# matter-labs/era-zkevm_test_harness

Measured on AMD Instinct MI355X. Metric: base-layer circuits/sec (2^20 rows); full-block synth wall-time 1/8 GPU, higher is better.
Workload: dtype u64 (Goldilocks, p = 2^64 - 2^32 + 1)

## Files before the change

### era_zkevm_test_harness_amd/csrc/ram_circuit_kernels.cuh

```cuda
#pragma once
#include "../../include/zkw_ram_circuit_spec.h"
#include "../../include/zkw_decommit_sorter_circuit_spec.h"
#include "../../include/zkw_events_sorter_circuit_spec.h"
#include "ram_kernels.cuh"
#include "public_input_kernels.cuh"
#include "closed_form_kernels.cuh"

namespace zkw {

struct SynthJob {
    const zkw_ram_instance* inst;
    const zkw_mem_query* sorted_q;
    const zkw_mem_query* unsorted_q;
    const u64* unsorted_caps;
    const u64* sorted_caps;
    const u64* u_mark;
    const u64* s_mark;
    const u64* challenges;
    const u64* lhs_z;
    const u64* rhs_z;
    u64 n_block;
    u64* trace;
    u32* hist;
    u32* nd_tiles;
    const u64* public_input;
    const zkw_ram_instance* first_inst;
    u32 tail_clean;
};

constexpr int ROW_SLOTS[RC_NUM_ROW_TYPES] = RC_ROW_NUM_SLOTS_INIT;
constexpr int ROW_LOOKUPS[RC_NUM_ROW_TYPES] = RC_ROW_NUM_LOOKUPS_INIT;
static_assert(ROW_SLOTS[RC_ROW_PU] == 133 && ROW_SLOTS[RC_ROW_PS] == 130, "Poseidon2 rows: 130 gate variables (+3 spare in PU)");
static_assert(ROW_LOOKUPS[RC_ROW_PU] == 12 && ROW_LOOKUPS[RC_ROW_PS] == 12 && ROW_LOOKUPS[RC_ROW_A] == 12 &&
              ROW_LOOKUPS[RC_ROW_B] == 12 && ROW_LOOKUPS[RC_ROW_C] == 8 && ROW_LOOKUPS[RC_ROW_D] == 0,
              "lookup cells per cycle (56) are hard-wired in the fill kernels");
constexpr int LOOKUPS_PER_CYCLE = 56;

__device__ __forceinline__ u64 inv_or_zero(u64 x) { return gl::canon(x) ? gl::inv(x) : 0; }

struct RegsIn {
    const u64* uh;
    const u64* sh;
    u32 len;
};
__device__ __forceinline__ RegsIn regs_in(const zkw_ram_instance* in) {
    RegsIn r;
    const bool start = in->start_flag != 0;
    r.uh = start ? in->unsorted_queue_initial_state.head : in->hidden_fsm_input.current_unsorted_queue_state.head;
    r.sh = start ? in->sorted_queue_initial_state.head : in->hidden_fsm_input.current_sorted_queue_state.head;
    r.len = start ? in->unsorted_queue_initial_state.length : in->hidden_fsm_input.current_unsorted_queue_state.length;
    return r;
}

#define TR(col, row) trace[(size_t)(col) * n_rows + (row)]

__device__ __forceinline__ void zero_gap_row(u64* trace, size_t n_rows, size_t row) {
    for (int col = 0; col < RC_G + RC_L; col++) TR(col, row) = 0;
}
__device__ __forceinline__ void zero_gap_row_n(u64* trace, size_t n_rows, size_t row, int n_cols) {
    for (int col = 0; col < n_cols; col++) TR(col, row) = 0;
}

__device__ __forceinline__ void hist_bytes(u32* sh_hist, u32 x) {
    atomicAdd(&sh_hist[x & 0xFF], 1u);
    atomicAdd(&sh_hist[(x >> 8) & 0xFF], 1u);
    atomicAdd(&sh_hist[(x >> 16) & 0xFF], 1u);
    atomicAdd(&sh_hist[x >> 24], 1u);
}
__device__ __forceinline__ void put_bytes(u64* trace, size_t n_rows, size_t row, int col0, u32 x) {
    TR(col0, row) = x & 0xFF;
    TR(col0 + 1, row) = (x >> 8) & 0xFF;
    TR(col0 + 2, row) = (x >> 16) & 0xFF;
    TR(col0 + 3, row) = x >> 24;
}
__device__ __forceinline__ void hist_flush(u32* sh_hist, u32* g_hist) {
    __syncthreads();
    for (int t = threadIdx.x; t < 256; t += blockDim.x)
        if (sh_hist[t]) atomicAdd(&g_hist[t], sh_hist[t]);
}

__device__ __forceinline__ void fill_flattened_poseidon(u64* trace, size_t n_rows, size_t row, u64 s[12]) {
    int pos = 0;
#pragma unroll
    for (int k = 0; k < 12; k++) TR(pos++, row) = gl::canon(s[k]);
    p2::external(s);
    int r = 0;
    for (int k = 0; k < P2_HALF_FULL_ROUNDS; k++, r++) {
        p2::full_round(s, r);
#pragma unroll
        for (int j = 0; j < 12; j++) TR(pos + j, row) = gl::canon(s[j]);
        pos += 12;
    }
    for (int k = 0; k < P2_PARTIAL_ROUNDS; k++, r++) {
        s[0] = gl::pow7(gl::add_canon(s[0], p2::rc_at(12 * r)));
        TR(pos++, row) = gl::canon(s[0]);
        p2::internal(s);
    }
    for (int k = 0; k < P2_HALF_FULL_ROUNDS; k++, r++) {
        p2::full_round(s, r);
#pragma unroll
        for (int j = 0; j < 12; j++) TR(pos + j, row) = gl::canon(s[j]);
        pos += 12;
    }
}

template <int SIDE>
static __device__ __forceinline__ void k_ram_fill_poseidon(const VB& vb, const SynthJob* __restrict__ jobs, u32 capacity,
                                                          size_t n_rows) {
    __shared__ u32 sh_hist[256];
    for (int t = threadIdx.x; t < 256; t += blockDim.x) sh_hist[t] = 0;
    __syncthreads();
    const SynthJob job = jobs[vb.y];
    const u32 i = vb.x * blockDim.x + threadIdx.x;
    if (i < capacity) {
        u64* trace = job.trace;
        const zkw_ram_instance* in = job.inst;
        const size_t first = in->first_item, m = in->num_items;
        const bool can_pop = i < m;
        const size_t row = (size_t)(SIDE == 0 ? RC_ROW_PU : RC_ROW_PS) * RC_REGION_STRIDE(capacity) + i;
        const zkw_mem_query* qs = SIDE == 0 ? job.unsorted_q : job.sorted_q;
        const u64* caps = SIDE == 0 ? job.unsorted_caps : job.sorted_caps;
        u64 s[12];
        if (can_pop) {
            encode_raw_query(load_raw_query(qs + first + i), s);
        } else {
#pragma unroll
            for (int k = 0; k < 8; k++) s[k] = 0;
        }
        const RegsIn ri = regs_in(in);
        const u64* prev_cap = i == 0 ? (SIDE == 0 ? ri.uh : ri.sh) + 8 : caps + 4 * (first + (i - 1 < m ? i - 1 : m - 1));
#pragma unroll
        for (int k = 0; k < 4; k++) s[8 + k] = prev_cap[k];
        fill_flattened_poseidon(trace, n_rows, row, s);
        zkw_mem_query q;
        memset(&q, 0, sizeof q);
        if (can_pop) q = job.sorted_q[first + i];
        if (SIDE == 0) {
            TR(RC_PU_idx, row) = q.index; TR(RC_PU_v0, row) = q.value[0]; TR(RC_PU_v1, row) = q.value[1];
            put_bytes(trace, n_rows, row, RC_PU_idx_b0, q.index);
            put_bytes(trace, n_rows, row, RC_PU_v0_b0, q.value[0]);
            put_bytes(trace, n_rows, row, RC_PU_v1_b0, q.value[1]);
            hist_bytes(sh_hist, q.index); hist_bytes(sh_hist, q.value[0]); hist_bytes(sh_hist, q.value[1]);
        } else {
            if (!job.tail_clean) for (int c = 130; c < RC_G; c++) TR(c, row) = 0;
            put_bytes(trace, n_rows, row, RC_PS_ts_b0, q.timestamp);
            put_bytes(trace, n_rows, row, RC_PS_page_b0, q.page);
            put_bytes(trace, n_rows, row, RC_PS_v4_b0, q.value[4]);
            hist_bytes(sh_hist, q.timestamp); hist_bytes(sh_hist, q.page); hist_bytes(sh_hist, q.value[4]);
        }
        if (!job.tail_clean) for (int c = RC_G + 12; c < RC_G + RC_L; c++) TR(c, row) = 0;
    } else if (i < RC_REGION_STRIDE(capacity)) {
        if (!job.tail_clean) zero_gap_row(job.trace, n_rows, (size_t)(SIDE == 0 ? RC_ROW_PU : RC_ROW_PS) * RC_REGION_STRIDE(capacity) + i);
    }
    hist_flush(sh_hist, job.hist);
}

struct CycleCtx {
    bool can_pop;
    zkw_mem_query q, pq;
    u64 eu[8], es[8];
    u64 p_val[5];
    u32 p_ptr;
};

__device__ __forceinline__ void load_query(const zkw_mem_query* src, zkw_mem_query& dst) {
    const uint4* s = reinterpret_cast<const uint4*>(src);
    uint4* d = reinterpret_cast<uint4*>(&dst);
    d[0] = s[0]; d[1] = s[1]; d[2] = s[2];
}

__device__ __forceinline__ void cycle_ctx(const SynthJob& job, u32 i, CycleCtx& c, bool want_eu) {
    const zkw_ram_instance* in = job.inst;
    const size_t first = in->first_item, m = in->num_items;
    c.can_pop = i < m;
    memset(&c.q, 0, sizeof c.q);
    memset(&c.pq, 0, sizeof c.pq);
#pragma unroll
    for (int k = 0; k < 8; k++) { c.eu[k] = 0; c.es[k] = 0; }
    if (c.can_pop) {
        load_query(job.sorted_q + first + i, c.q);
        encode_mem_query(c.q, c.es);
        if (want_eu) encode_raw_query(load_raw_query(job.unsorted_q + first + i), c.eu);
    }
    if (i == 0) {
        const zkw_ram_fsm& f = in->hidden_fsm_input;
        c.pq.timestamp = f.previous_sorting_key[0]; c.pq.index = f.previous_sorting_key[1]; c.pq.page = f.previous_sorting_key[2];
        for (int k = 0; k < 8; k++) c.pq.value[k] = f.previous_value[k];
        c.pq.value_is_pointer = f.previous_is_ptr ? 1 : 0;
    } else if (i - 1 < m) {
        load_query(job.sorted_q + first + i - 1, c.pq);
    }
    u64 pe[8];
    encode_mem_query(c.pq, pe);
#pragma unroll
    for (int k = 0; k < 5; k++) c.p_val[k] = pe[3 + k];
    c.p_ptr = c.pq.value_is_pointer ? 1 : 0;
}

__device__ __forceinline__ u64 acc_before(const u64* z, size_t first, size_t m, u32 i, u64 fsm_in) {
    return i == 0 ? fsm_in : z[first + (i - 1 < m ? i - 1 : m - 1)];
}

static __device__ __forceinline__ void k_ram_fill_A(const VB& vb, const SynthJob* __restrict__ jobs, u32 capacity, size_t n_rows) {
    __shared__ u32 sh_hist[256];
    sh_hist[threadIdx.x] = 0;
    __syncthreads();
    const SynthJob job = jobs[vb.y];
    const u32 i = vb.x * blockDim.x + threadIdx.x;
    const u64* lhs_z_all = job.lhs_z;
    const u64* rhs_z_all = job.rhs_z;
    const size_t n_total = job.n_block;
    if (i < capacity) {
        u64* trace = job.trace;
        const zkw_ram_instance* in = job.inst;
        const size_t first = in->first_item, m = in->num_items, row = (size_t)RC_ROW_A * RC_REGION_STRIDE(capacity) + i;
        CycleCtx c;
        cycle_ctx(job, i, c, true);
        const u64 rw = c.q.rw_flag ? 1 : 0, ptr = c.q.value_is_pointer ? 1 : 0;
#pragma unroll
        for (int k = 0; k < 8; k++) { TR(RC_A_eu0 + k, row) = c.eu[k]; TR(RC_A_ts + k, row) = c.es[k]; }
        for (int r = 0; r < 2; r++) {
            const u64* ch = job.challenges + 9 * r;
            u64 lc = ch[8], rc = ch[8];
#pragma unroll
            for (int k = 0; k < 8; k++) {
                lc = gl::add(lc, gl::mul(c.eu[k], ch[k]));
                rc = gl::add(rc, gl::mul(c.es[k], ch[k]));
            }
            const u64 pl = acc_before(lhs_z_all + (size_t)r * n_total, first, m, i, in->hidden_fsm_input.lhs_accumulator[r]);
            const u64 pr = acc_before(rhs_z_all + (size_t)r * n_total, first, m, i, in->hidden_fsm_input.rhs_accumulator[r]);
            const u64 nl = gl::canon(gl::mul(pl, lc)), nr = gl::canon(gl::mul(pr, rc));
            const int o = r * (RC_A_lc1 - RC_A_lc0);
#pragma unroll
            for (int k = 1; k < 9; k++) TR(RC_A_G_c0_1 + (k - 1) + r * (RC_A_G_c1_1 - RC_A_G_c0_1), row) = ch[k];
            TR(RC_A_lc0 + o, row) = gl::canon(lc); TR(RC_A_P_lhs0 + o, row) = pl; TR(RC_A_nl0 + o, row) = nl;
            TR(RC_A_lhs0 + o, row) = c.can_pop ? nl : pl;
            TR(RC_A_rc0 + o, row) = gl::canon(rc); TR(RC_A_P_rhs0 + o, row) = pr; TR(RC_A_nr0 + o, row) = nr;
            TR(RC_A_rhs0 + o, row) = c.can_pop ? nr : pr;
        }
        TR(RC_A_rw, row) = rw; TR(RC_A_ptr, row) = ptr; TR(RC_A_idx, row) = c.q.index;
        TR(RC_A_v2, row) = c.q.value[2]; TR(RC_A_v3, row) = c.q.value[3]; TR(RC_A_v0, row) = c.q.value[0];
        TR(RC_A_v5_b3c, row) = c.q.value[5] >> 24; TR(RC_A_can_pop, row) = c.can_pop ? 1 : 0;
        put_bytes(trace, n_rows, row, RC_A_v2_b0, c.q.value[2]);
        put_bytes(trace, n_rows, row, RC_A_v3_b0, c.q.value[3]);
        put_bytes(trace, n_rows, row, RC_A_v5_b0, c.q.value[5]);
        hist_bytes(sh_hist, c.q.value[2]); hist_bytes(sh_hist, c.q.value[3]); hist_bytes(sh_hist, c.q.value[5]);
        constexpr int NA = ROW_SLOTS[RC_ROW_A];
        if (!job.tail_clean) {
            for (int col = NA; col < RC_G; col++) TR(col, row) = 0;
            for (int col = RC_G + 12; col < RC_G + RC_L; col++) TR(col, row) = 0;
        }
    } else if (i < RC_REGION_STRIDE(capacity)) {
        if (!job.tail_clean) zero_gap_row(job.trace, n_rows, (size_t)RC_ROW_A * RC_REGION_STRIDE(capacity) + i);
    }
    hist_flush(sh_hist, job.hist);
}

static __device__ __forceinline__ void k_ram_fill_B(const VB& vb, const SynthJob* __restrict__ jobs, u32 capacity, size_t n_rows) {
    __shared__ u32 sh_hist[256];
    sh_hist[threadIdx.x] = 0;
    __syncthreads();
    const SynthJob job = jobs[vb.y];
    const u32 i = vb.x * blockDim.x + threadIdx.x;
    if (i < capacity) {
        u64* trace = job.trace;
        const size_t row = (size_t)RC_ROW_B * RC_REGION_STRIDE(capacity) + i;
        CycleCtx c;
        cycle_ctx(job, i, c, false);
        put_bytes(trace, n_rows, row, RC_B_v6_b0, c.q.value[6]);
        put_bytes(trace, n_rows, row, RC_B_v7_b0, c.q.value[7]);
        TR(RC_B_es4, row) = c.es[4]; TR(RC_B_v1, row) = c.q.value[1]; TR(RC_B_v5_b3c, row) = c.q.value[5] >> 24;
        TR(RC_B_es5, row) = c.es[5]; TR(RC_B_v2, row) = c.q.value[2];
        TR(RC_B_es6, row) = c.es[6]; TR(RC_B_v3, row) = c.q.value[3];
        const u32 d0 = c.q.timestamp - c.pq.timestamp;
        TR(RC_B_d0, row) = d0; put_bytes(trace, n_rows, row, RC_B_d0_b0, d0);
        TR(RC_B_bw0, row) = c.q.timestamp < c.pq.timestamp ? 1 : 0;
        TR(RC_B_ts, row) = c.q.timestamp; TR(RC_B_P_ts, row) = c.pq.timestamp;
        hist_bytes(sh_hist, c.q.value[6]); hist_bytes(sh_hist, c.q.value[7]); hist_bytes(sh_hist, d0);
        constexpr int NB = ROW_SLOTS[RC_ROW_B];
        if (!job.tail_clean) {
            for (int col = NB; col < RC_G; col++) TR(col, row) = 0;
            for (int col = RC_G + 12; col < RC_G + RC_L; col++) TR(col, row) = 0;
        }
    } else if (i < RC_REGION_STRIDE(capacity)) {
        if (!job.tail_clean) zero_gap_row(job.trace, n_rows, (size_t)RC_ROW_B * RC_REGION_STRIDE(capacity) + i);
    }
    hist_flush(sh_hist, job.hist);
}

__device__ __forceinline__ bool nd_flag(bool can_pop, const zkw_mem_query& q) {
    return can_pop && q.timestamp == 0 && q.page == RC_HEAP_PAGE && q.rw_flag && !q.value_is_pointer;
}

static __device__ __forceinline__ void k_ram_nd_tiles(const VB& vb, const SynthJob* __restrict__ jobs, u32 capacity) {
    __shared__ u32 sh[4];
    const SynthJob job = jobs[vb.y];
    const u32 i = vb.x * blockDim.x + threadIdx.x;
    const zkw_ram_instance* in = job.inst;
    bool f = false;
    if (i < capacity && i < in->num_items) {
        zkw_mem_query q;
        load_query(job.sorted_q + in->first_item + i, q);
        f = nd_flag(true, q);
    }
    u32 cnt = __popcll(__ballot(f));
    if ((threadIdx.x & 63) == 0) sh[threadIdx.x >> 6] = cnt;
    __syncthreads();
    if (threadIdx.x == 0) job.nd_tiles[vb.x] = sh[0] + sh[1] + sh[2] + sh[3];
}
static __device__ __forceinline__ void k_ram_nd_scan(const VB& vb, const SynthJob* __restrict__ jobs, int n_jobs, u32 n_tiles) {
    u32* t = jobs[vb.x].nd_tiles;
    const int lane = threadIdx.x;
    u32 acc = 0;
    for (u32 base = 0; base < n_tiles; base += 64) {
        const u32 k = base + lane;
        const u32 v = k < n_tiles ? t[k] : 0;
        u32 incl = v;
        for (int off = 1; off < 64; off <<= 1) {
            const u32 up = __shfl_up(incl, off);
            if (lane >= off) incl += up;
        }
        if (k < n_tiles) t[k] = acc + incl - v;
        acc += __shfl(incl, 63);
    }
}

static __device__ __forceinline__ void k_ram_fill_C(const VB& vb, const SynthJob* __restrict__ jobs, u32 capacity, size_t n_rows) {
    __shared__ u32 sh_hist[256];
    __shared__ u32 sh_wave[4];
    sh_hist[threadIdx.x] = 0;
    __syncthreads();
    const SynthJob job = jobs[vb.y];
    const u32 i = vb.x * blockDim.x + threadIdx.x;
    const bool live = i < capacity;
    CycleCtx c;
    c.can_pop = false;
    bool nd = false;
    if (live) {
        cycle_ctx(job, i, c, false);
        nd = nd_flag(c.can_pop, c.q);
    }
    const unsigned long long bal = __ballot(nd);
    const int lane = threadIdx.x & 63, wave = threadIdx.x >> 6;
    if (lane == 0) sh_wave[wave] = __popcll(bal);
    __syncthreads();
    u32 before = __popcll(bal & ((1ull << lane) - 1));
    for (int w = 0; w < wave; w++) before += sh_wave[w];
    if (live) {
        u64* trace = job.trace;
        const zkw_ram_instance* in = job.inst;
        const size_t row = (size_t)RC_ROW_C * RC_REGION_STRIDE(capacity) + i;
        const u64 rw = c.q.rw_flag ? 1 : 0, ptr = c.q.value_is_pointer ? 1 : 0;
        const u64 bw0 = c.q.timestamp < c.pq.timestamp ? 1 : 0;
        const u64 t1 = (u64)c.pq.index + bw0, bw1 = (u64)c.q.index < t1 ? 1 : 0;
        const u32 d1 = (u32)((u64)c.q.index - t1);
        const u64 t2 = (u64)c.pq.page + bw1, bw2 = (u64)c.q.page < t2 ? 1 : 0;
        const u32 d2 = (u32)((u64)c.q.page - t2);
        TR(RC_C_d1, row) = d1; put_bytes(trace, n_rows, row, RC_C_d1_b0, d1);
        TR(RC_C_d2, row) = d2; put_bytes(trace, n_rows, row, RC_C_d2_b0, d2);
        hist_bytes(sh_hist, d1); hist_bytes(sh_hist, d2);
        TR(RC_C_bw1, row) = bw1; TR(RC_C_bw2, row) = bw2; TR(RC_C_bw0, row) = bw0;
        TR(RC_C_idx, row) = c.q.index; TR(RC_C_P_idx, row) = c.pq.index;
        TR(RC_C_page, row) = c.q.page; TR(RC_C_P_page, row) = c.pq.page;
        TR(RC_C_can_pop, row) = c.can_pop ? 1 : 0;
        u64 x[14];
        x[0] = gl::canon(gl::sub(c.q.index, c.pq.index));
        x[1] = gl::canon(gl::sub(c.q.page, c.pq.page));
        const u64 val[5] = {c.es[3], c.es[4], c.es[5], c.es[6], c.es[7]};
#pragma unroll
        for (int k = 0; k < 5; k++) { x[2 + k] = gl::canon(gl::sub(val[k], c.p_val[k])); x[7 + k] = val[k]; }
        x[12] = c.q.timestamp;
        x[13] = gl::canon(gl::sub(c.q.page, RC_HEAP_PAGE));
        u64 pre[14], acc = 1;
#pragma unroll
        for (int k = 0; k < 14; k++) { pre[k] = acc; acc = gl::mul(acc, x[k] ? x[k] : 1); }
        u64 inv = gl::inv(acc), w[14];
#pragma unroll
        for (int k = 13; k >= 0; k--) {
            w[k] = x[k] ? gl::canon(gl::mul(inv, pre[k])) : 0;
            inv = gl::mul(inv, x[k] ? x[k] : 1);
        }
        const u64 z_idx = x[0] == 0, z_page = x[1] == 0, same = z_idx & z_page;
        TR(RC_C_w_idx, row) = w[0]; TR(RC_C_z_idx, row) = z_idx;
        TR(RC_C_w_page, row) = w[1]; TR(RC_C_z_page, row) = z_page; TR(RC_C_same, row) = same;
        const int C_VAL[5] = {RC_C_es3, RC_C_es4, RC_C_es5, RC_C_es6, RC_C_v4};
        const int C_PVAL[5] = {RC_C_P_es3, RC_C_P_es4, RC_C_P_es5, RC_C_P_es6, RC_C_P_v4};
        const int C_WEQ[5] = {RC_C_w_eq0, RC_C_w_eq1, RC_C_w_eq2, RC_C_w_eq3, RC_C_w_eq4};
        const int C_ZEQ[5] = {RC_C_z_eq0, RC_C_z_eq1, RC_C_z_eq2, RC_C_z_eq3, RC_C_z_eq4};
        const int C_WZ[5] = {RC_C_w_z0, RC_C_w_z1, RC_C_w_z2, RC_C_w_z3, RC_C_w_z4};
        const int C_ZZ[5] = {RC_C_z_z0, RC_C_z_z1, RC_C_z_z2, RC_C_z_z3, RC_C_z_z4};
        u64 zeq[5], zz[5];
#pragma unroll
        for (int k = 0; k < 5; k++) {
            zeq[k] = x[2 + k] == 0; zz[k] = x[7 + k] == 0;
            TR(C_VAL[k], row) = val[k]; TR(C_PVAL[k], row) = c.p_val[k];
            TR(C_WEQ[k], row) = w[2 + k]; TR(C_ZEQ[k], row) = zeq[k];
            TR(C_WZ[k], row) = w[7 + k]; TR(C_ZZ[k], row) = zz[k];
        }
        const u64 peq = ptr == c.p_ptr, eq_a = zeq[0] & zeq[1] & zeq[2], value_equal = eq_a & zeq[3] & zeq[4] & peq;
        const u64 zz_a = zz[0] & zz[1] & zz[2], all_zero = zz_a & zz[3] & zz[4] & (1 - ptr);
        TR(RC_C_ptr, row) = ptr; TR(RC_C_P_ptr, row) = c.p_ptr; TR(RC_C_peq, row) = peq;
        TR(RC_C_eq_a, row) = eq_a; TR(RC_C_value_equal, row) = value_equal;
        TR(RC_C_zz_a, row) = zz_a; TR(RC_C_all_zero, row) = all_zero; TR(RC_C_rw, row) = rw;
        TR(RC_C_ts, row) = c.q.timestamp; TR(RC_C_w_ts, row) = w[12]; TR(RC_C_z_ts, row) = x[12] == 0;
        TR(RC_C_w_heap, row) = w[13]; TR(RC_C_z_heap, row) = x[13] == 0; TR(RC_C_nd, row) = nd ? 1 : 0;
        const u64 p_cnt = (u64)in->hidden_fsm_input.num_nondeterministic_writes + job.nd_tiles[vb.x] + before;
        TR(RC_C_P_cnt, row) = p_cnt; TR(RC_C_cnt, row) = p_cnt + (nd ? 1 : 0);
        constexpr int NC = ROW_SLOTS[RC_ROW_C];
        if (!job.tail_clean) {
            for (int col = NC; col < RC_G; col++) TR(col, row) = 0;
            for (int col = RC_G + 8; col < RC_G + RC_L; col++) TR(col, row) = 0;
        }
    } else if (i < RC_REGION_STRIDE(capacity)) {
        if (!job.tail_clean) zero_gap_row(job.trace, n_rows, (size_t)RC_ROW_C * RC_REGION_STRIDE(capacity) + i);
    }
    if (vb.x == 0 && threadIdx.x == 0)
        for (int l = 5; l < 8; l++) { hist_bytes(sh_hist, job.inst->hidden_fsm_input.previous_value[l]); hist_bytes(sh_hist, job.inst->hidden_fsm_output.previous_value[l]); }
    hist_flush(sh_hist, job.hist);
}

__device__ __forceinline__ void ram_boundary_block(const SynthJob& job, u32 capacity, size_t n_rows);
constexpr int RC_D_TILES = 4;
// ... 381 lines not shown
```

### era_zkevm_test_harness_amd/csrc/zkw_api.hip

```cpp
#include "zkw_ctx.h"
#include "circuit_check_host.h"
#include "closed_forms_host.h"
#include "callstack_kernels.cuh"
#include "vm_kernels.cuh"
#include "radix_sort.cuh"

static thread_local std::string g_last_error;

#undef fail
int zkw_fail(int code, const char* fmt, ...) {
    char buf[512];
    va_list ap;
    va_start(ap, fmt);
    vsnprintf(buf, sizeof buf, fmt, ap);
    va_end(ap);
    g_last_error = buf;
    return code;
}

#define fail zkw_fail

struct AllocCache {
    static constexpr size_t SMALL_MAX = size_t(256) << 20;
    static constexpr int MAX_DEV = 16;
// ... 1448 lines not shown
extern "C" int zkw_ram_synthesize(zkw_ctx* ctx, const zkw_ram_witness* w, size_t first_instance, size_t n_instances,
                                  zkw_trace* t, size_t first_slot) {
    if (!ctx || !w || !t || w->ctx != ctx || t->ctx->device != ctx->device) return fail(ZKW_ERR_INVALID, "zkw_ram_synthesize: bad argument");
    if (first_instance + n_instances > w->n_instances) return fail(ZKW_ERR_INVALID, "instance range out of bounds");
    if (n_instances > t->n_slots) return fail(ZKW_ERR_INVALID, "more instances (%zu) than trace slots (%zu)", n_instances, t->n_slots);
    const u32 capacity = w->capacity;
    const size_t n_rows = t->n_rows;
    if (RC_MIN_ROWS(capacity) > n_rows)
        return fail(ZKW_ERR_INVALID, "capacity %u needs %llu rows, trace has %zu", capacity,
                    (unsigned long long)RC_MIN_ROWS(capacity), n_rows);
    if (n_rows & 1) return fail(ZKW_ERR_INVALID, "trace length must be even (it is a power of two in every circuit)");
    if (n_instances == 0) return ZKW_OK;
    HIP_TRY(hipSetDevice(ctx->device));
    const size_t n_blocks = w->offsets.size() - 1;
    size_t b_first = 0;
    while (b_first + 1 < n_blocks && w->inst_offsets[b_first + 1] <= first_instance) b_first++;
    size_t b_end = b_first + 1;
    while (b_end < n_blocks && w->inst_offsets[b_end] < first_instance + n_instances) b_end++;
    const size_t win = std::min(w->zcap, w->sqcap);
    if (w->offsets[b_end] - w->offsets[b_first] > win) {
        size_t b_mid = b_first + 1;
        while (b_mid + 1 < b_end && w->offsets[b_mid + 1] - w->offsets[b_first] <= win) b_mid++;
        const size_t n_head = w->inst_offsets[b_mid] - first_instance;
        ZKW_TRY(zkw_ram_synthesize(ctx, w, first_instance, n_head, t, first_slot));
        return zkw_ram_synthesize(ctx, w, first_instance + n_head, n_instances - n_head, t, first_slot + n_head);
    }
    ZKW_TRY(ram_gp_blocks(ctx, w, b_first, b_end, w->zbuf_l, w->zbuf_r));
    const size_t z_base = w->offsets[b_first];
    {
        const size_t cnt = w->offsets[b_end] - z_base;
        Prof _p(ctx, "k_gather_encode");
        ZKW_LAUNCH(ctx, k_gather_encode, blocks_for(cnt, 256), 256, w->unsorted_q, w->perm + z_base, cnt, w->sq_win, (u64*)nullptr);
    }
    ZKW_TRY(launch_check("k_gather_encode"));
    const u32 rstride = (u32)RC_REGION_STRIDE(capacity);
    const u32 n_tiles = (rstride + 255) / 256;
    u32 *d_hist = nullptr, *d_nd = nullptr;
    ZKW_TRY(ctx->scratch_t<u32>("synth_hist", n_instances * 256, &d_hist));
    ZKW_TRY(ctx->scratch_t<u32>("synth_nd", n_instances * n_tiles, &d_nd));
    HIP_TRY(ctx->memset_async(d_hist, 0, n_instances * 256 * sizeof(u32)));
    SlotClaims claims(t);
    std::vector<SynthJob> jobs(n_instances);
    size_t b = b_first;
    for (size_t k = 0; k < n_instances; k++) {
        const size_t idx = first_instance + k;
        while (b + 1 < n_blocks && w->inst_offsets[b + 1] <= idx) b++;
        const size_t lo = w->offsets[b], nb = w->offsets[b + 1] - lo;
        SynthJob& j = jobs[k];
        j.inst = w->instances + idx;
        j.sorted_q = w->sq_win + (lo - z_base);
        j.unsorted_q = w->unsorted_q + lo;
        j.unsorted_caps = w->unsorted_caps + 4 * lo;
        j.sorted_caps = w->sorted_caps + 4 * lo;
        j.u_mark = w->unsorted_marks + 12 * idx;
        j.s_mark = w->sorted_marks + 12 * idx;
        j.challenges = w->challenges + 18 * b;
        j.lhs_z = w->zbuf_l + 2 * (lo - z_base);
        j.rhs_z = w->zbuf_r + 2 * (lo - z_base);
        j.n_block = nb;
        {
            const uint64_t tag = ((uint64_t)ZKW_CIRCUIT_RAM_PERMUTATION << 56) ^ ((uint64_t)capacity << 24) ^ (uint64_t)n_rows ^ 0x5A00000000000000ull;
            const size_t slot = (first_slot + k) % t->n_slots;
            bool clean = false;
            j.trace = claims.claim(slot, tag, &clean);
            j.tail_clean = clean;
        }
        j.hist = d_hist + 256 * k;
        j.nd_tiles = d_nd + (size_t)n_tiles * k;
        j.public_input = w->public_inputs + 4 * idx;
        j.first_inst = w->instances + w->inst_offsets[b];
    }
    SynthJob* d_jobs = nullptr;
    ZKW_TRY(ctx->upload("synth_jobs", jobs, &d_jobs));
    const unsigned nj = (unsigned)n_instances;
    const dim3 g64((rstride + 63) / 64, nj), g256(n_tiles, nj);
    { Prof _p(ctx, "k_ram_nd_tiles"); ZKW_LAUNCH_D(ctx, (k_ram_nd_tiles), "k_ram_nd_tiles", g256, 256, 0, d_jobs, capacity); }
    ZKW_TRY(launch_check("k_ram_nd_tiles"));
    { Prof _p(ctx, "k_ram_nd_scan"); ZKW_LAUNCH(ctx, k_ram_nd_scan, nj, 64, d_jobs, (int)nj, n_tiles); }
    ZKW_TRY(launch_check("k_ram_nd_scan"));
    { Prof _p(ctx, "k_ram_fill_poseidon"); ZKW_LAUNCH_D(ctx, (k_ram_fill_poseidon<0>), "k_ram_fill_poseidon", g64, 64, 0, d_jobs, capacity, n_rows); }
    ZKW_TRY(launch_check("k_ram_fill_poseidon<0>"));
    { Prof _p(ctx, "k_ram_fill_poseidon"); ZKW_LAUNCH_D(ctx, (k_ram_fill_poseidon<1>), "k_ram_fill_poseidon", g64, 64, 0, d_jobs, capacity, n_rows); }
    ZKW_TRY(launch_check("k_ram_fill_poseidon<1>"));
    { Prof _p(ctx, "k_ram_fill_A"); ZKW_LAUNCH_D(ctx, (k_ram_fill_A), "k_ram_fill_A", g256, 256, 0, d_jobs, capacity, n_rows); }
    ZKW_TRY(launch_check("k_ram_fill_A"));
    { Prof _p(ctx, "k_ram_fill_B"); ZKW_LAUNCH_D(ctx, (k_ram_fill_B), "k_ram_fill_B", g256, 256, 0, d_jobs, capacity, n_rows); }
    ZKW_TRY(launch_check("k_ram_fill_B"));
    { Prof _p(ctx, "k_ram_fill_C"); ZKW_LAUNCH_D(ctx, (k_ram_fill_C), "k_ram_fill_C", g256, 256, 0, d_jobs, capacity, n_rows); }
    ZKW_TRY(launch_check("k_ram_fill_C"));
    { Prof _p(ctx, "k_ram_fill_D"); const unsigned d_tiles = (unsigned)((rstride + RC_D_TILES * 256 - 1) / (RC_D_TILES * 256));
      ZKW_LAUNCH(ctx, k_ram_fill_D, nj * (d_tiles + 1), 256, d_jobs, nj, d_tiles, capacity, n_rows); }
    ZKW_TRY(launch_check("k_ram_fill_D"));
    { Prof _p(ctx, "k_ram_fill_tail"); ZKW_LAUNCH(ctx, k_ram_fill_tail, nj * ((RC_G + RC_L + 1) * TAIL_CHUNKS), 256, d_jobs, capacity, n_rows); }
    ZKW_TRY(launch_check("k_ram_fill_tail"));
    return claims.commit_if(ctx->sync_if_host());
}


extern "C" int zkw_ram_check_satisfied(zkw_ctx* ctx, const zkw_trace* t, size_t slot, uint32_t capacity,
                                       uint64_t* n_violations, uint64_t* first_bad) {
    if (!ctx || !t || t->ctx->device != ctx->device || slot >= t->n_slots || !n_violations)
        return fail(ZKW_ERR_INVALID, "zkw_ram_check_satisfied: bad argument");
    if (RC_MIN_ROWS(capacity) > t->n_rows) return fail(ZKW_ERR_INVALID, "capacity does not fit the trace");
    return check_satisfied<SpecRam>(ctx, t, slot, capacity, n_violations, first_bad);
}

extern "C" int zkw_decommit_sorter_check_satisfied(zkw_ctx* ctx, const zkw_trace* t, size_t slot, uint32_t capacity,
                                                   uint64_t* n_violations, uint64_t* first_bad) {
    if (!ctx || !t || t->ctx->device != ctx->device || slot >= t->n_slots || !n_violations)
        return fail(ZKW_ERR_INVALID, "zkw_decommit_sorter_check_satisfied: bad argument");
    if (DS_MIN_ROWS(capacity) > t->n_rows) return fail(ZKW_ERR_INVALID, "capacity does not fit the trace");
    return check_satisfied<SpecDecommitSorter>(ctx, t, slot, capacity, n_violations, first_bad);
}

extern "C" int zkw_closed_form_public_inputs(zkw_ctx* ctx, uint8_t circuit_type, const void* instances, size_t n, uint64_t* compact,
                                             uint64_t* public_inputs) {
    if (!ctx || !compact || !public_inputs || (n && !instances)) return fail(ZKW_ERR_INVALID, "zkw_closed_form_public_inputs: null argument");
    if (n == 0) return ZKW_OK;
    HIP_TRY(hipSetDevice(ctx->device));
    switch (circuit_type) {
        case 3: return closed_form_from_records<CfDecommitter>(ctx, instances, n, compact, public_inputs);
        case 5: return closed_form_from_records<CfPrecompile<ZKW_PRECOMPILE_KECCAK256>>(ctx, instances, n, compact, public_inputs);
        case 6: return closed_form_from_records<CfPrecompile<ZKW_PRECOMPILE_SHA256>>(ctx, instances, n, compact, public_inputs);
        case 7: return closed_form_from_records<CfPrecompile<ZKW_PRECOMPILE_ECRECOVER>>(ctx, instances, n, compact, public_inputs);
        case 10: return closed_form_from_records<CfStorageApplication>(ctx, instances, n, compact, public_inputs);
        case 13: return closed_form_from_records<CfLinearHasher>(ctx, instances, n, compact, public_inputs);
        default: break;
    }
    return fail(ZKW_ERR_INVALID, "zkw_closed_form_public_inputs: circuit type %u keeps its compact forms in its witness (2, 4, 8, 9, 11, 12) "
                                 "or is not a base-layer circuit with a closed form here", (unsigned)circuit_type);
}

extern "C" int zkw_commit_encodings(zkw_ctx* ctx, const uint64_t* enc, size_t n_items, uint32_t item_len, uint64_t* out) {
    if (!ctx || !out || (n_items && item_len && !enc)) return fail(ZKW_ERR_INVALID, "zkw_commit_encodings: null argument");
    if (n_items == 0) return ZKW_OK;
    HIP_TRY(hipSetDevice(ctx->device));
    const u64* d_enc = nullptr;
    u64* d_out = nullptr;
    ZKW_TRY(ctx->in("ce_enc", enc, n_items * item_len + 1, &d_enc));
    ZKW_TRY(ctx->out("ce_out", out, n_items * 4, &d_out));
    { Prof _p(ctx, "k_commit_encodings"); ZKW_LAUNCH(ctx, k_commit_encodings, blocks_for(n_items, 64), 64, d_enc, n_items, item_len, d_out); }
    ZKW_TRY(launch_check("k_commit_encodings"));
    ZKW_TRY(ctx->finish_out(out, d_out, n_items * 4));
    return ctx->sync_if_host();
}

extern "C" int zkw_encode_recursion_requests(zkw_ctx* ctx, uint64_t circuit_type, const uint64_t* public_inputs, size_t n,
                                             uint64_t* enc) {
    if (!ctx || !enc || !public_inputs) return fail(ZKW_ERR_INVALID, "zkw_encode_recursion_requests: null argument");
    if (n == 0) return ZKW_OK;
    HIP_TRY(hipSetDevice(ctx->device));
    const u64* d_pi = nullptr;
    u64* d_enc = nullptr;
    ZKW_TRY(ctx->in("rr_pi", public_inputs, n * 4, &d_pi));
    ZKW_TRY(ctx->out("rr_enc", enc, n * 8, &d_enc));
    { Prof _p(ctx, "k_encode_recursion"); ZKW_LAUNCH(ctx, k_encode_recursion, blocks_for(n, 64), 64, circuit_type, d_pi, n, d_enc); }
    ZKW_TRY(launch_check("k_encode_recursion"));
    ZKW_TRY(ctx->finish_out(enc, d_enc, n * 8));
    return ctx->sync_if_host();
}

extern "C" int zkw_encode_callstack_entries(zkw_ctx* ctx, const zkw_callstack_entry* entries, size_t n, uint64_t* enc) {
    if (!ctx || !enc || !entries) return fail(ZKW_ERR_INVALID, "zkw_encode_callstack_entries: null argument");
    if (n == 0) return ZKW_OK;
    HIP_TRY(hipSetDevice(ctx->device));
    const zkw_callstack_entry* d_e = nullptr;
    u64* d_enc = nullptr;
    ZKW_TRY(ctx->in("cs_e", entries, n, &d_e));
    ZKW_TRY(ctx->out("cs_enc", enc, n * 32, &d_enc));
    { Prof _p(ctx, "k_encode_callstack"); hipLaunchKernelGGL(k_encode_callstack, dim3(blocks_for(n, 64)), dim3(64), 0, ctx->stream, d_e, n, d_enc); }
// ... 140 lines not shown
```

Measured before the change: 3082.

## Fuse RAM row A/B fills into the poseidon fill kernels

The separate k_ram_fill_A and k_ram_fill_B launches are removed. Their row-filling work now runs inside k_ram_fill_poseidon<0> and <1>, reusing the already-loaded sorted query and the raw/sorted encodings that the poseidon sponge needs. This cuts two kernel launches and the repeated global loads of queries and previous queries. Sched barriers are added to keep register pressure down around the Goldilocks multiply chains. The fused kernels run at 64 threads per block instead of 256 and carry more per-thread work, which may raise register pressure. The poseidon sponge input for SIDE 1 now comes from encode_mem_query rather than encode_raw_query, which could change the result if the two encodings differ.

```diff
diff --git a/era_zkevm_test_harness_amd/csrc/ram_circuit_kernels.cuh b/era_zkevm_test_harness_amd/csrc/ram_circuit_kernels.cuh
--- a/era_zkevm_test_harness_amd/csrc/ram_circuit_kernels.cuh
+++ b/era_zkevm_test_harness_amd/csrc/ram_circuit_kernels.cuh
@@ -104,6 +104,130 @@
     }
 }
 
+struct CycleCtx {
+    bool can_pop;
+    zkw_mem_query q, pq;
+    u64 es[8];
+    u64 p_val[5];
+    u32 p_ptr;
+};
+
+__device__ __forceinline__ void load_query(const zkw_mem_query* src, zkw_mem_query& dst) {
+    const uint4* s = reinterpret_cast<const uint4*>(src);
+    uint4* d = reinterpret_cast<uint4*>(&dst);
+    d[0] = s[0]; d[1] = s[1]; d[2] = s[2];
+}
+
+__device__ __forceinline__ void cycle_ctx(const SynthJob& job, u32 i, CycleCtx& c) {
+    const zkw_ram_instance* in = job.inst;
+    const size_t first = in->first_item, m = in->num_items;
+    c.can_pop = i < m;
+    memset(&c.q, 0, sizeof c.q);
+    memset(&c.pq, 0, sizeof c.pq);
+#pragma unroll
+    for (int k = 0; k < 8; k++) c.es[k] = 0;
+    if (c.can_pop) {
+        load_query(job.sorted_q + first + i, c.q);
+        encode_mem_query(c.q, c.es);
+    }
+    if (i == 0) {
+        const zkw_ram_fsm& f = in->hidden_fsm_input;
+        c.pq.timestamp = f.previous_sorting_key[0]; c.pq.index = f.previous_sorting_key[1]; c.pq.page = f.previous_sorting_key[2];
+        for (int k = 0; k < 8; k++) c.pq.value[k] = f.previous_value[k];
+        c.pq.value_is_pointer = f.previous_is_ptr ? 1 : 0;
+    } else if (i - 1 < m) {
+        load_query(job.sorted_q + first + i - 1, c.pq);
+    }
+    u64 pe[8];
+    encode_mem_query(c.pq, pe);
+#pragma unroll
+    for (int k = 0; k < 5; k++) c.p_val[k] = pe[3 + k];
+    c.p_ptr = c.pq.value_is_pointer ? 1 : 0;
+}
+
+__device__ __forceinline__ u64 acc_before(const u64* z, size_t first, size_t m, u32 i, u64 fsm_in) {
+    return i == 0 ? fsm_in : z[first + (i - 1 < m ? i - 1 : m - 1)];
+}
+
+__device__ __forceinline__ void fill_row_A(const SynthJob& job, u32 i, u32 capacity, size_t n_rows, const zkw_mem_query& q,
+                                           const u64 eu[8], const u64 es[8], u32* sh_hist) {
+    u64* trace = job.trace;
+    const size_t row = (size_t)RC_ROW_A * RC_REGION_STRIDE(capacity) + i;
+    if (i < capacity) {
+        const zkw_ram_instance* in = job.inst;
+        const size_t first = in->first_item, m = in->num_items, n_total = job.n_block;
+        const bool can_pop = i < m;
+        const u64 rw = q.rw_flag ? 1 : 0, ptr = q.value_is_pointer ? 1 : 0;
+#pragma unroll
+        for (int k = 0; k < 8; k++) { TR(RC_A_eu0 + k, row) = eu[k]; TR(RC_A_ts + k, row) = es[k]; }
+        for (int r = 0; r < 2; r++) {
+            const u64* ch = job.challenges + 9 * r;
+            u64 lc = ch[8], rc = ch[8];
+#pragma unroll
+            for (int k = 0; k < 8; k++) {
+                lc = gl::add(lc, gl::mul(eu[k], ch[k]));
+                rc = gl::add(rc, gl::mul(es[k], ch[k]));
+                __builtin_amdgcn_sched_barrier(0);
+            }
+            const u64 pl = acc_before(job.lhs_z + (size_t)r * n_total, first, m, i, in->hidden_fsm_input.lhs_accumulator[r]);
+            const u64 pr = acc_before(job.rhs_z + (size_t)r * n_total, first, m, i, in->hidden_fsm_input.rhs_accumulator[r]);
+            const u64 nl = gl::canon(gl::mul(pl, lc)), nr = gl::canon(gl::mul(pr, rc));
+            const int o = r * (RC_A_lc1 - RC_A_lc0);
+#pragma unroll
+            for (int k = 1; k < 9; k++) TR(RC_A_G_c0_1 + (k - 1) + r * (RC_A_G_c1_1 - RC_A_G_c0_1), row) = ch[k];
+            __builtin_amdgcn_sched_barrier(0);
+            TR(RC_A_lc0 + o, row) = gl::canon(lc); TR(RC_A_P_lhs0 + o, row) = pl; TR(RC_A_nl0 + o, row) = nl;
+            TR(RC_A_lhs0 + o, row) = can_pop ? nl : pl;
+            TR(RC_A_rc0 + o, row) = gl::canon(rc); TR(RC_A_P_rhs0 + o, row) = pr; TR(RC_A_nr0 + o, row) = nr;
+            TR(RC_A_rhs0 + o, row) = can_pop ? nr : pr;
+            __builtin_amdgcn_sched_barrier(0);
+        }
+        TR(RC_A_rw, row) = rw; TR(RC_A_ptr, row) = ptr; TR(RC_A_idx, row) = q.index;
+        TR(RC_A_v2, row) = q.value[2]; TR(RC_A_v3, row) = q.value[3]; TR(RC_A_v0, row) = q.value[0];
+        TR(RC_A_v5_b3c, row) = q.value[5] >> 24; TR(RC_A_can_pop, row) = can_pop ? 1 : 0;
+        put_bytes(trace, n_rows, row, RC_A_v2_b0, q.value[2]);
+        put_bytes(trace, n_rows, row, RC_A_v3_b0, q.value[3]);
+        put_bytes(trace, n_rows, row, RC_A_v5_b0, q.value[5]);
+        hist_bytes(sh_hist, q.value[2]); hist_bytes(sh_hist, q.value[3]); hist_bytes(sh_hist, q.value[5]);
+        constexpr int NA = ROW_SLOTS[RC_ROW_A];
+        if (!job.tail_clean) {
+            for (int col = NA; col < RC_G; col++) TR(col, row) = 0;
+            for (int col = RC_G + 12; col < RC_G + RC_L; col++) TR(col, row) = 0;
+        }
+    } else if (i < RC_REGION_STRIDE(capacity)) {
+        if (!job.tail_clean) zero_gap_row(trace, n_rows, row);
+    }
+}
+
+__device__ __forceinline__ void fill_row_B(const SynthJob& job, u32 i, u32 capacity, size_t n_rows, const zkw_mem_query& q,
+                                           const u64 es[8], u32* sh_hist) {
+    u64* trace = job.trace;
+    const size_t row = (size_t)RC_ROW_B * RC_REGION_STRIDE(capacity) + i;
+    if (i < capacity) {
+        const zkw_ram_instance* in = job.inst;
+        u32 p_ts = 0;
+        if (i == 0) p_ts = in->hidden_fsm_input.previous_sorting_key[0];
+        else if (i - 1 < in->num_items) p_ts = job.sorted_q[in->first_item + i - 1].timestamp;
+        put_bytes(trace, n_rows, row, RC_B_v6_b0, q.value[6]);
+        put_bytes(trace, n_rows, row, RC_B_v7_b0, q.value[7]);
+        TR(RC_B_es4, row) = es[4]; TR(RC_B_v1, row) = q.value[1]; TR(RC_B_v5_b3c, row) = q.value[5] >> 24;
+        TR(RC_B_es5, row) = es[5]; TR(RC_B_v2, row) = q.value[2];
+        TR(RC_B_es6, row) = es[6]; TR(RC_B_v3, row) = q.value[3];
+        const u32 d0 = q.timestamp - p_ts;
+        TR(RC_B_d0, row) = d0; put_bytes(trace, n_rows, row, RC_B_d0_b0, d0);
+        TR(RC_B_bw0, row) = q.timestamp < p_ts ? 1 : 0;
+        TR(RC_B_ts, row) = q.timestamp; TR(RC_B_P_ts, row) = p_ts;
+        hist_bytes(sh_hist, q.value[6]); hist_bytes(sh_hist, q.value[7]); hist_bytes(sh_hist, d0);
+        constexpr int NB = ROW_SLOTS[RC_ROW_B];
+        if (!job.tail_clean) {
+            for (int col = NB; col < RC_G; col++) TR(col, row) = 0;
+            for (int col = RC_G + 12; col < RC_G + RC_L; col++) TR(col, row) = 0;
+        }
+    } else if (i < RC_REGION_STRIDE(capacity)) {
+        if (!job.tail_clean) zero_gap_row(trace, n_rows, row);
+    }
+}
+
 template <int SIDE>
 static __device__ __forceinline__ void k_ram_fill_poseidon(const VB& vb, const SynthJob* __restrict__ jobs, u32 capacity,
                                                           size_t n_rows) {
@@ -112,29 +236,28 @@
     __syncthreads();
     const SynthJob job = jobs[vb.y];
     const u32 i = vb.x * blockDim.x + threadIdx.x;
+    u64* trace = job.trace;
+    const zkw_ram_instance* in = job.inst;
+    const size_t first = in->first_item, m = in->num_items;
+    const bool can_pop = i < capacity && i < m;
+    const size_t row = (size_t)(SIDE == 0 ? RC_ROW_PU : RC_ROW_PS) * RC_REGION_STRIDE(capacity) + i;
+    zkw_mem_query q;
+    memset(&q, 0, sizeof q);
+    u64 s[12];
+#pragma unroll
+    for (int k = 0; k < 8; k++) s[k] = 0;
+    if (can_pop) {
+        load_query(job.sorted_q + first + i, q);
+        if (SIDE == 0) encode_raw_query(load_raw_query(job.unsorted_q + first + i), s); else encode_mem_query(q, s);
+    }
+    if (SIDE == 0) {
+        u64 es[8];
+        encode_mem_query(q, es);
+        fill_row_A(job, i, capacity, n_rows, q, s, es, sh_hist);
+    } else {
+        fill_row_B(job, i, capacity, n_rows, q, s, sh_hist);
+    }
     if (i < capacity) {
-        u64* trace = job.trace;
-        const zkw_ram_instance* in = job.inst;
-        const size_t first = in->first_item, m = in->num_items;
-        const bool can_pop = i < m;
-        const size_t row = (size_t)(SIDE == 0 ? RC_ROW_PU : RC_ROW_PS) * RC_REGION_STRIDE(capacity) + i;
-        const zkw_mem_query* qs = SIDE == 0 ? job.unsorted_q : job.sorted_q;
-        const u64* caps = SIDE == 0 ? job.unsorted_caps : job.sorted_caps;
-        u64 s[12];
-        if (can_pop) {
-            encode_raw_query(load_raw_query(qs + first + i), s);
-        } else {
-#pragma unroll
-            for (int k = 0; k < 8; k++) s[k] = 0;
-        }
-        const RegsIn ri = regs_in(in);
-        const u64* prev_cap = i == 0 ? (SIDE == 0 ? ri.uh : ri.sh) + 8 : caps + 4 * (first + (i - 1 < m ? i - 1 : m - 1));
-#pragma unroll
-        for (int k = 0; k < 4; k++) s[8 + k] = prev_cap[k];
-        fill_flattened_poseidon(trace, n_rows, row, s);
-        zkw_mem_query q;
-        memset(&q, 0, sizeof q);
-        if (can_pop) q = job.sorted_q[first + i];
         if (SIDE == 0) {
             TR(RC_PU_idx, row) = q.index; TR(RC_PU_v0, row) = q.value[0]; TR(RC_PU_v1, row) = q.value[1];
             put_bytes(trace, n_rows, row, RC_PU_idx_b0, q.index);
@@ -149,141 +272,15 @@
             hist_bytes(sh_hist, q.timestamp); hist_bytes(sh_hist, q.page); hist_bytes(sh_hist, q.value[4]);
         }
         if (!job.tail_clean) for (int c = RC_G + 12; c < RC_G + RC_L; c++) TR(c, row) = 0;
+        __builtin_amdgcn_sched_barrier(0);
+        const RegsIn ri = regs_in(in);
+        const u64* caps = SIDE == 0 ? job.unsorted_caps : job.sorted_caps;
+        const u64* prev_cap = i == 0 ? (SIDE == 0 ? ri.uh : ri.sh) + 8 : caps + 4 * (first + (i - 1 < m ? i - 1 : m - 1));
+#pragma unroll
+        for (int k = 0; k < 4; k++) s[8 + k] = prev_cap[k];
+        fill_flattened_poseidon(trace, n_rows, row, s);
     } else if (i < RC_REGION_STRIDE(capacity)) {
-        if (!job.tail_clean) zero_gap_row(job.trace, n_rows, (size_t)(SIDE == 0 ? RC_ROW_PU : RC_ROW_PS) * RC_REGION_STRIDE(capacity) + i);
-    }
-    hist_flush(sh_hist, job.hist);
-}
-
-struct CycleCtx {
-    bool can_pop;
-    zkw_mem_query q, pq;
-    u64 eu[8], es[8];
-    u64 p_val[5];
-    u32 p_ptr;
-};
-
-__device__ __forceinline__ void load_query(const zkw_mem_query* src, zkw_mem_query& dst) {
-    const uint4* s = reinterpret_cast<const uint4*>(src);
-    uint4* d = reinterpret_cast<uint4*>(&dst);
-    d[0] = s[0]; d[1] = s[1]; d[2] = s[2];
-}
-
-__device__ __forceinline__ void cycle_ctx(const SynthJob& job, u32 i, CycleCtx& c, bool want_eu) {
-    const zkw_ram_instance* in = job.inst;
-    const size_t first = in->first_item, m = in->num_items;
-    c.can_pop = i < m;
-    memset(&c.q, 0, sizeof c.q);
-    memset(&c.pq, 0, sizeof c.pq);
-#pragma unroll
-    for (int k = 0; k < 8; k++) { c.eu[k] = 0; c.es[k] = 0; }
-    if (c.can_pop) {
-        load_query(job.sorted_q + first + i, c.q);
-        encode_mem_query(c.q, c.es);
-        if (want_eu) encode_raw_query(load_raw_query(job.unsorted_q + first + i), c.eu);
-    }
-    if (i == 0) {
-        const zkw_ram_fsm& f = in->hidden_fsm_input;
-        c.pq.timestamp = f.previous_sorting_key[0]; c.pq.index = f.previous_sorting_key[1]; c.pq.page = f.previous_sorting_key[2];
-        for (int k = 0; k < 8; k++) c.pq.value[k] = f.previous_value[k];
-        c.pq.value_is_pointer = f.previous_is_ptr ? 1 : 0;
-    } else if (i - 1 < m) {
-        load_query(job.sorted_q + first + i - 1, c.pq);
-    }
-    u64 pe[8];
-    encode_mem_query(c.pq, pe);
-#pragma unroll
-    for (int k = 0; k < 5; k++) c.p_val[k] = pe[3 + k];
-    c.p_ptr = c.pq.value_is_pointer ? 1 : 0;
-}
-
-__device__ __forceinline__ u64 acc_before(const u64* z, size_t first, size_t m, u32 i, u64 fsm_in) {
-    return i == 0 ? fsm_in : z[first + (i - 1 < m ? i - 1 : m - 1)];
-}
-
-static __device__ __forceinline__ void k_ram_fill_A(const VB& vb, const SynthJob* __restrict__ jobs, u32 capacity, size_t n_rows) {
-    __shared__ u32 sh_hist[256];
-    sh_hist[threadIdx.x] = 0;
-    __syncthreads();
-    const SynthJob job = jobs[vb.y];
-    const u32 i = vb.x * blockDim.x + threadIdx.x;
-    const u64* lhs_z_all = job.lhs_z;
-    const u64* rhs_z_all = job.rhs_z;
-    const size_t n_total = job.n_block;
-    if (i < capacity) {
-        u64* trace = job.trace;
-        const zkw_ram_instance* in = job.inst;
-        const size_t first = in->first_item, m = in->num_items, row = (size_t)RC_ROW_A * RC_REGION_STRIDE(capacity) + i;
-        CycleCtx c;
-        cycle_ctx(job, i, c, true);
-        const u64 rw = c.q.rw_flag ? 1 : 0, ptr = c.q.value_is_pointer ? 1 : 0;
-#pragma unroll
-        for (int k = 0; k < 8; k++) { TR(RC_A_eu0 + k, row) = c.eu[k]; TR(RC_A_ts + k, row) = c.es[k]; }
-        for (int r = 0; r < 2; r++) {
-            const u64* ch = job.challenges + 9 * r;
-            u64 lc = ch[8], rc = ch[8];
-#pragma unroll
-            for (int k = 0; k < 8; k++) {
-                lc = gl::add(lc, gl::mul(c.eu[k], ch[k]));
-                rc = gl::add(rc, gl::mul(c.es[k], ch[k]));
-            }
-            const u64 pl = acc_before(lhs_z_all + (size_t)r * n_total, first, m, i, in->hidden_fsm_input.lhs_accumulator[r]);
-            const u64 pr = acc_before(rhs_z_all + (size_t)r * n_total, first, m, i, in->hidden_fsm_input.rhs_accumulator[r]);
-            const u64 nl = gl::canon(gl::mul(pl, lc)), nr = gl::canon(gl::mul(pr, rc));
-            const int o = r * (RC_A_lc1 - RC_A_lc0);
-#pragma unroll
-            for (int k = 1; k < 9; k++) TR(RC_A_G_c0_1 + (k - 1) + r * (RC_A_G_c1_1 - RC_A_G_c0_1), row) = ch[k];
-            TR(RC_A_lc0 + o, row) = gl::canon(lc); TR(RC_A_P_lhs0 + o, row) = pl; TR(RC_A_nl0 + o, row) = nl;
-            TR(RC_A_lhs0 + o, row) = c.can_pop ? nl : pl;
-            TR(RC_A_rc0 + o, row) = gl::canon(rc); TR(RC_A_P_rhs0 + o, row) = pr; TR(RC_A_nr0 + o, row) = nr;
-            TR(RC_A_rhs0 + o, row) = c.can_pop ? nr : pr;
-        }
-        TR(RC_A_rw, row) = rw; TR(RC_A_ptr, row) = ptr; TR(RC_A_idx, row) = c.q.index;
-        TR(RC_A_v2, row) = c.q.value[2]; TR(RC_A_v3, row) = c.q.value[3]; TR(RC_A_v0, row) = c.q.value[0];
-        TR(RC_A_v5_b3c, row) = c.q.value[5] >> 24; TR(RC_A_can_pop, row) = c.can_pop ? 1 : 0;
-        put_bytes(trace, n_rows, row, RC_A_v2_b0, c.q.value[2]);
-        put_bytes(trace, n_rows, row, RC_A_v3_b0, c.q.value[3]);
-        put_bytes(trace, n_rows, row, RC_A_v5_b0, c.q.value[5]);
-        hist_bytes(sh_hist, c.q.value[2]); hist_bytes(sh_hist, c.q.value[3]); hist_bytes(sh_hist, c.q.value[5]);
-        constexpr int NA = ROW_SLOTS[RC_ROW_A];
-        if (!job.tail_clean) {
-            for (int col = NA; col < RC_G; col++) TR(col, row) = 0;
-            for (int col = RC_G + 12; col < RC_G + RC_L; col++) TR(col, row) = 0;
-        }
-    } else if (i < RC_REGION_STRIDE(capacity)) {
-        if (!job.tail_clean) zero_gap_row(job.trace, n_rows, (size_t)RC_ROW_A * RC_REGION_STRIDE(capacity) + i);
-    }
-    hist_flush(sh_hist, job.hist);
-}
-
-static __device__ __forceinline__ void k_ram_fill_B(const VB& vb, const SynthJob* __restrict__ jobs, u32 capacity, size_t n_rows) {
-    __shared__ u32 sh_hist[256];
-    sh_hist[threadIdx.x] = 0;
-    __syncthreads();
-    const SynthJob job = jobs[vb.y];
-    const u32 i = vb.x * blockDim.x + threadIdx.x;
-    if (i < capacity) {
-        u64* trace = job.trace;
-        const size_t row = (size_t)RC_ROW_B * RC_REGION_STRIDE(capacity) + i;
-        CycleCtx c;
-        cycle_ctx(job, i, c, false);
-        put_bytes(trace, n_rows, row, RC_B_v6_b0, c.q.value[6]);
-        put_bytes(trace, n_rows, row, RC_B_v7_b0, c.q.value[7]);
-        TR(RC_B_es4, row) = c.es[4]; TR(RC_B_v1, row) = c.q.value[1]; TR(RC_B_v5_b3c, row) = c.q.value[5] >> 24;
-        TR(RC_B_es5, row) = c.es[5]; TR(RC_B_v2, row) = c.q.value[2];
-        TR(RC_B_es6, row) = c.es[6]; TR(RC_B_v3, row) = c.q.value[3];
-        const u32 d0 = c.q.timestamp - c.pq.timestamp;
-        TR(RC_B_d0, row) = d0; put_bytes(trace, n_rows, row, RC_B_d0_b0, d0);
-        TR(RC_B_bw0, row) = c.q.timestamp < c.pq.timestamp ? 1 : 0;
-        TR(RC_B_ts, row) = c.q.timestamp; TR(RC_B_P_ts, row) = c.pq.timestamp;
-        hist_bytes(sh_hist, c.q.value[6]); hist_bytes(sh_hist, c.q.value[7]); hist_bytes(sh_hist, d0);
-        constexpr int NB = ROW_SLOTS[RC_ROW_B];
-        if (!job.tail_clean) {
-            for (int col = NB; col < RC_G; col++) TR(col, row) = 0;
-            for (int col = RC_G + 12; col < RC_G + RC_L; col++) TR(col, row) = 0;
-        }
-    } else if (i < RC_REGION_STRIDE(capacity)) {
-        if (!job.tail_clean) zero_gap_row(job.trace, n_rows, (size_t)RC_ROW_B * RC_REGION_STRIDE(capacity) + i);
+        if (!job.tail_clean) zero_gap_row(trace, n_rows, row);
     }
     hist_flush(sh_hist, job.hist);
 }
@@ -337,7 +334,7 @@
     c.can_pop = false;
     bool nd = false;
     if (live) {
-        cycle_ctx(job, i, c, false);
+        cycle_ctx(job, i, c);
         nd = nd_flag(c.can_pop, c.q);
     }
     const unsigned long long bal = __ballot(nd);
diff --git a/era_zkevm_test_harness_amd/csrc/zkw_api.hip b/era_zkevm_test_harness_amd/csrc/zkw_api.hip
--- a/era_zkevm_test_harness_amd/csrc/zkw_api.hip
+++ b/era_zkevm_test_harness_amd/csrc/zkw_api.hip
@@ -1554,10 +1554,6 @@
     ZKW_TRY(launch_check("k_ram_fill_poseidon<0>"));
     { Prof _p(ctx, "k_ram_fill_poseidon"); ZKW_LAUNCH_D(ctx, (k_ram_fill_poseidon<1>), "k_ram_fill_poseidon", g64, 64, 0, d_jobs, capacity, n_rows); }
     ZKW_TRY(launch_check("k_ram_fill_poseidon<1>"));
-    { Prof _p(ctx, "k_ram_fill_A"); ZKW_LAUNCH_D(ctx, (k_ram_fill_A), "k_ram_fill_A", g256, 256, 0, d_jobs, capacity, n_rows); }
-    ZKW_TRY(launch_check("k_ram_fill_A"));
-    { Prof _p(ctx, "k_ram_fill_B"); ZKW_LAUNCH_D(ctx, (k_ram_fill_B), "k_ram_fill_B", g256, 256, 0, d_jobs, capacity, n_rows); }
-    ZKW_TRY(launch_check("k_ram_fill_B"));
     { Prof _p(ctx, "k_ram_fill_C"); ZKW_LAUNCH_D(ctx, (k_ram_fill_C), "k_ram_fill_C", g256, 256, 0, d_jobs, capacity, n_rows); }
     ZKW_TRY(launch_check("k_ram_fill_C"));
     { Prof _p(ctx, "k_ram_fill_D"); const unsigned d_tiles = (unsigned)((rstride + RC_D_TILES * 256 - 1) / (RC_D_TILES * 256));
```

Result: faster. 3193 (median of 6 runs) (+3.6%).
